# PASSIONLab/ELBA

Measured on AMD Instinct MI355X. Metric: overlap nnz/sec (A·Aᵀ SpGEMM, SharedSeeds semiring, after Prune(numshared<=1)), higher is better.
Workload: dtype u32

## Files before the change

### elba_amd/csrc/ov_plan.hpp

```cpp
#pragma once
#include <algorithm>
#include <cstddef>
#include <cstdint>

namespace elba {

constexpr int NUM_LDS_TIERS = 5;
constexpr int NUM_TIERS = NUM_LDS_TIERS + 1;
constexpr int LDS_TBITS0 = 9;
constexpr uint32_t STAGE_CHUNK = 1024;
constexpr uint32_t STAGE_REC_BYTES = 32;
constexpr uint32_t FIN_WAVE2_MAX = 1024;
constexpr uint32_t SLAB_PAD = 16;
constexpr int RP_TILE = 1024;
constexpr int FIN_HUGE_BLOCKS = 32;
constexpr int OV_SAMPLE_ROWS = 256, OV_SAMPLE_TIER = 3;
constexpr size_t OV_LDS_MAX = 160 * 1024;

namespace ov_spec {
constexpr uint32_t half = 1, inl = 1, pay16 = 1, rec16 = 1, suffix = 0, qblk_log2 = 0, j_shift = 0;
constexpr uint32_t hint_mask = 1u << 31, pos_mask = 0x3FFFFFFFu;
}

enum OvFamily { OV_DENSE, OV_PAY, OV_S32, OV_SHARED };
// ... 11 lines not shown
    {OV_PAY, 2, 512, 11, 0, 2, 26, false, true, false, 0},
    {OV_PAY, 3, 1024, 12, 0, 1, 26, false, true, false, 0},
    {OV_S32, 0, 128, 9, 0, 12, 18, false, false, false, 0},
    {OV_S32, 1, 256, 10, 0, 7, 18, false, false, false, 0},
    {OV_S32, 2, 512, 11, 0, 3, 18, false, false, false, 0},
    {OV_S32, 3, 1024, 12, 0, 1, 18, false, false, false, 0},
    {OV_SHARED, 4, 256, 13, 0, 1, 18, false, false, false, 0},
    {OV_SHARED, NUM_LDS_TIERS, 256, 0, 0, OV_GRID_SPILL, 0, true, false, false, 0},
};
constexpr int OV_NROWS = (int)(sizeof(OV_ROWS) / sizeof(OV_ROWS[0]));

constexpr int64_t ov_stage_slack(int num_cus) { return (int64_t)num_cus * 32 * STAGE_CHUNK + 64; }

constexpr size_t ov_row_lds(const OvTierRow &r, bool pay16)
{
    const size_t waves = (size_t)(r.block / 64), table = r.global ? 0 : (size_t)r.slot_bytes << r.tbits;
    return table + 256 + waves * (r.dense ? 2368 : r.global ? 2560 : r.payload ? 3072 : pay16 ? 2048 : 2560);
}

inline int ov_row_of(OvFamily family, int tier, int dense_up)
{
    int found = -1;
    for (int r = 0; r < OV_NROWS; ++r) {
        const OvTierRow &x = OV_ROWS[r];
        if (x.tier == tier && (x.family == family || x.family == OV_SHARED) && dense_up >= x.dense_up_min) found = r;
    }
    return found;
}

struct OvOptions {
    bool no_symmetry = false, no_pay = false, mir32 = false, no_slab = false, no_sample = false, ov_generic = false;
    int dk = -1, dense_up = 1, dense_wgs = 8, slab_q16 = 0, slab_pct = 175;
    int64_t tune3 = 0, tune4 = 0, tune5 = 0, tune7 = 0;
};
struct OvHints { uint32_t prior_q16 = 0, slab_q16 = 0; bool tiers_known = false, tier_used[NUM_TIERS] = {false, false, false, false, false, false}, sort_used[2] = {false, false}; };
struct OvInput {
    int64_t M = 0, N = 0, Z = 0, row_lo = 0, row_hi = 0, max_row_nnz = 0, max_col_nnz = 0;
    uint32_t fbits = 1;
    bool pos16 = false, use_ell = false, csr_hints = false, csr_inline = false, csr_suffix = false, have_row_order = false;
    int num_cus = 256;
    OvOptions opt;
    OvHints hints;
    int phase = 0, pass = 1;
    int64_t tmp_cap = 0, free_bytes = 0, workspace_hint_bytes = 0;
};

struct OvLaunch { int row = -1, grid = 0, block = 0; size_t lds = 0; };
struct OvFinPlan {
    int64_t nrows = 0;
    bool slabs = false, scan_rowptr = false, narrow = false;
    int slab_fold_blocks = 0, rowptr_blocks = 0, row_blocks = 0, bucket_blocks = 0, huge_blocks = FIN_HUGE_BLOCKS;
    uint64_t sort_stride = 2;
    uint32_t sorts = 0;
};
struct OvPlan {
    int64_t nrows = 0;
    bool whole = false, ell = false, forced = false;
    uint32_t half = 0, pos_mask = 0, hint_mask = 0, suffix = 0, inl = 0;
    bool row_order = false, hints_used = false;
    bool pay = false, pay16 = false;
    OvFamily family = OV_S32;
    int dk = 1;
    bool spec = false;
    uint32_t min_tier = 0, qblk_log2 = 0, prior_q16 = 16384, use_feedback = 1, max_col = 1;
    unsigned long long fb_enough = 0;
    uint32_t nsample = 0, sstep = 1;
    bool slab_on = false; int64_t slab_cap = 0; uint32_t slab_prior_q16 = 0;
    uint64_t gstride = 2; int spill_blocks = 64;
    int64_t slack = 0, tmp_cap = 0, b_cap = 0;
    bool mir16 = false;
    uint32_t tier_limit[NUM_LDS_TIERS] = {0, 0, 0, 0, 0};
    OvLaunch tier[NUM_TIERS], sample;
    int tmax = NUM_TIERS;
    uint32_t launched = 0;
    int zero_blocks_max = 0, classify_blocks = 0;
    OvFinPlan fin;
};

inline bool ov_spec_ok(const OvPlan &p)
{
    return !p.forced && p.dk == 0 && !p.pay && (p.pay16 ? 1u : 0u) == ov_spec::pay16 && p.ell && p.half == ov_spec::half && p.hint_mask == ov_spec::hint_mask &&
           p.pos_mask == ov_spec::pos_mask && p.inl == ov_spec::inl && (p.mir16 ? 1u : 0u) == ov_spec::rec16 && p.suffix == ov_spec::suffix && !p.row_order &&
           p.qblk_log2 == ov_spec::qblk_log2 && p.whole;
}

inline OvLaunch ov_launch_of(int row, bool pay16, int num_cus, int dense_wgs, int spill_blocks)
{
    const OvTierRow &r = OV_ROWS[row];
    OvLaunch l;
    l.row = row; l.block = r.block; l.lds = ov_row_lds(r, pay16);
    l.grid = r.cu_factor == OV_GRID_SPILL ? spill_blocks : num_cus * (r.cu_factor == OV_GRID_DENSE_WGS ? dense_wgs : r.cu_factor);
    return l;
}

inline OvFinPlan plan_ov_finalize(const OvInput &in, bool slabs, bool all_sorts, bool remote)
{
    OvFinPlan f;
    const int64_t M = in.M, cus = in.num_cus;
    f.nrows = in.row_hi - in.row_lo;
    f.slabs = slabs;
    f.slab_fold_blocks = slabs && f.nrows > 0 ? (int)((f.nrows + 255) / 256) : 0;
    while (f.sort_stride < (uint64_t)M) f.sort_stride <<= 1;
    f.scan_rowptr = M + 1 > (1 << 17);
    f.rowptr_blocks = (int)(f.scan_rowptr ? (M + 1 + 255) / 256 : (M + 1 + RP_TILE - 1) / RP_TILE);
    if (f.nrows <= 0) return f;
    f.row_blocks = (int)std::min<int64_t>((f.nrows + 3) / 4, cus * 32);
    f.narrow = in.opt.tune4 != 2 && !remote &&
               std::min<uint64_t>((uint64_t)std::max<int64_t>(in.max_row_nnz, 1) * (uint64_t)std::max<int64_t>(in.max_col_nnz, 1), (uint64_t)M) <= (uint64_t)FIN_WAVE2_MAX;
    f.bucket_blocks = (int)std::min<int64_t>(f.nrows, cus * 4);
    if (!f.narrow && (all_sorts || in.hints.sort_used[0])) f.sorts |= 1u;
    if (!f.narrow && (all_sorts || in.hints.sort_used[1])) f.sorts |= 2u;
    return f;
}

inline bool ov_one_triangle(const OvInput &in) { return in.phase >= 1 || !in.opt.no_symmetry || in.csr_inline; }

struct OvSpill { uint64_t gstride; int blocks; };
inline OvSpill ov_spill_tables(int64_t M, int num_cus)
{
    OvSpill s{2, 0};
    while (s.gstride < 2ull * (uint64_t)(M > 1 ? M : 1)) s.gstride <<= 1;
    s.blocks = (int)((4ull << 30) / (20ull * s.gstride));
    s.blocks = s.blocks < 64 ? 64 : (s.blocks > num_cus * 2 ? num_cus * 2 : s.blocks);
    return s;
}

inline void ov_plan_capacities(const OvInput &in, OvPlan &p)
{
    const int64_t M = in.M, Z = in.Z;
    const bool half = ov_one_triangle(in);
    const OvSpill sp = ov_spill_tables(M, in.num_cus);
    p.gstride = sp.gstride; p.spill_blocks = sp.blocks;
    p.slack = ov_stage_slack(in.num_cus);
    p.tmp_cap = in.tmp_cap;
    if (p.tmp_cap == 0) {
        if (in.workspace_hint_bytes > 0) p.tmp_cap = in.workspace_hint_bytes / (int64_t)STAGE_REC_BYTES;
        else {
            const int64_t budget = (int64_t)((size_t)in.free_bytes / 2 / (STAGE_REC_BYTES + (half ? 2 * (24 + 32) : 24)));
            p.tmp_cap = std::min<int64_t>(std::max<int64_t>(half ? Z / 2 : Z, 1 << 16) + p.slack, std::max<int64_t>(budget, 1024));
        }
        if (p.tmp_cap < 1024) p.tmp_cap = 1024;
    }
    p.b_cap = half ? 2 * p.tmp_cap : p.tmp_cap;
}

inline void ov_plan_switches(const OvInput &in, OvPlan &p)
{
    const OvOptions &o = in.opt;
    const int64_t Z = in.Z, nrows = p.nrows;
    p.max_col = (uint32_t)(in.max_col_nnz > 0 ? in.max_col_nnz : 1);
    p.half = in.phase >= 1 ? 2u : (ov_one_triangle(in) ? 1u : 0u);
    p.pos_mask = in.csr_suffix ? 0xFFFFu : (in.csr_hints ? 0x3FFFFFFFu : 0xFFFFFFFFu);
    p.hint_mask = !in.csr_hints ? 0u : (p.half == 2u ? 1u << 30 : (p.half == 1u ? 1u << 31 : 0u));
    p.suffix = in.csr_suffix && p.half == 1u ? 1u : 0u;
    p.inl = in.csr_inline ? 1u : 0u;
    p.row_order = p.suffix && in.have_row_order;
    p.hints_used = p.hint_mask != 0u || p.suffix != 0u || in.csr_inline;
    p.prior_q16 = in.hints.prior_q16 ? in.hints.prior_q16 : 16384u;
    p.use_feedback = in.hints.prior_q16 ? 0u : 1u;
    p.fb_enough = (unsigned long long)std::min<int64_t>(std::max<int64_t>(Z / 32, 1 << 16), 1 << 23);
    p.pay = in.pos16 && !o.no_pay;
    p.pay16 = p.pay && in.use_ell && !in.csr_suffix && o.tune3 != 1 && ((uint64_t)in.max_row_nnz << in.fbits) <= 65536ull;
// ... 96 lines not shown
```

### elba_amd/csrc/spgemm.hip

```cpp
#include "common.hpp"
#include "ov_plan.hpp"
#include <algorithm>
#include <string>
#include <type_traits>
#include <utility>

namespace elba {

namespace {

constexpr uint32_t EMPTY = 0xFFFFFFFFu;
constexpr uint32_t FIN_WAVE_MAX = 256;
constexpr uint32_t FIN_LDS_MAX = 4096;

struct alignas(128) OvShard {
    unsigned long long yraw, nnz, ndiag, nupper, fb_claims, fb_ub, products;
    unsigned int maxshared;
    unsigned int tier_done[NUM_TIERS];
};
constexpr int NUM_SHARDS = 64;

struct OvCounters {
    unsigned long long cursor;
    unsigned long long products;
// ... 74 lines not shown
    uint32_t tier_limit[NUM_LDS_TIERS];
    unsigned long long fb_enough, tmp_cap;
    uint32_t *row_cnt, *low_cnt; unsigned long long *row_off;
    uint32_t *lists, *sample_list;
    OvCounters *ctr;
    uint4 *rec; uint32_t *tick;
    uint4 *slab; unsigned long long *slab_pos;
};

struct ZeroList { uint32_t *p[6]; size_t words[6]; int n; };
__global__ __launch_bounds__(256) void k_zero_regions(ZeroList z)
{
    const size_t stride = (size_t)gridDim.x * 256u;
    for (int q = 0; q < z.n; ++q)
        for (size_t i = (size_t)blockIdx.x * 256u + threadIdx.x; i < z.words[q]; i += stride) z.p[q][i] = 0u;
}

struct __attribute__((packed, aligned(4))) RowPair { uint32_t a, b; };
__device__ __forceinline__ uint32_t slab_base(uint32_t rp, uint32_t rp0, uint32_t row_rel, uint32_t q16)
{
    return (uint32_t)(((unsigned long long)(rp - rp0) * q16) >> 16) + SLAB_PAD * row_rel;
}

__device__ __forceinline__ uint32_t wave_sum_u32(uint32_t v)
{
#pragma unroll
    for (int d = 32; d >= 1; d >>= 1) v += __shfl_xor(v, d, 64);
    return v;
}

__device__ __forceinline__ uint32_t guaranteed_tbits(uint32_t ub, uint32_t mcols)
{
    const uint32_t need = ub < mcols ? ub : mcols;
    return need <= 1 ? 1u : (uint32_t)(32 - __clz(2 * need - 1));
}

#include "spgemm_table.hpp"
#include "spgemm_direct.hpp"

struct FinParams {
    const uint32_t *row_cnt; uint32_t *low_cnt; const unsigned long long *row_off; int64_t *b_rowptr;
    const StageRec *tmp; StageRec *mir;
    uint32_t rec16; const uint4 *rec; const uint32_t *tick;
    uint32_t *b_col; elba_seed_t *b_val;
    uint32_t M, row_lo, row_hi, half;
    uint32_t *fin_lists; OvCounters *ctr;
    uint64_t *sortkeys; unsigned long long sort_stride;
    uint32_t *sum_tmp;
    long long b_cap;
    uint32_t mir16;
    const uint32_t *tick_rows;
    const uint32_t *a_rowptr; uint4 *slab;
    const unsigned long long *slab_pos; uint32_t *slab_n;
};

struct SlabCall { uint32_t q16, rp0; };
__device__ __forceinline__ SlabCall slab_call(const FinParams &p)
{
    SlabCall s{0u, 0u};
    if (p.slab) { s.q16 = p.ctr->slab_q16; if (s.q16) s.rp0 = p.a_rowptr[p.row_lo]; }
    return s;
}
__device__ __forceinline__ uint2 slab_row(const FinParams &p, const SlabCall &s, uint32_t i)
{
    if (!s.q16) return make_uint2(0u, 0u);
    return make_uint2(slab_base(p.a_rowptr[i], s.rp0, i - p.row_lo, s.q16), p.slab_n[i]);
}
__global__ void k_slab_fold(FinParams p)
{
    const uint32_t i = p.row_lo + blockIdx.x * blockDim.x + threadIdx.x;
    if (i >= p.row_hi) return;
    const SlabCall s = slab_call(p);
    uint32_t n = 0;
    if (s.q16) {
        const unsigned long long w = p.slab_pos[i];
        const uint32_t base = slab_base(p.a_rowptr[i], s.rp0, i - p.row_lo, s.q16), cur = (uint32_t)w, lim = (uint32_t)(w >> 32);
        n = (cur < lim ? cur : lim) - base;
    }
    p.slab_n[i] = n;
}

__device__ __forceinline__ void fin_load(const FinParams &p, uint32_t low, unsigned long long off, int64_t dst, uint32_t t, uint4 &a, uint4 &b, uint2 sl = make_uint2(0u, 0u))
{
    if (t >= low) {
        if (p.rec16) {
            const uint4 m = p.rec[off + (t - low)];
            a = make_uint4(m.x, 0xFFFFFFFFu, m.y & 0xFFFFu, m.y >> 16); b = make_uint4(m.z & 0xFFFFu, m.z >> 16, m.w, 0u);
        } else { const StageRec *r = &p.tmp[off + (t - low)]; a = r->a; b = r->b; }
    }
    else if (p.mir16) {
        const uint4 m = t < sl.y ? p.slab[sl.x + t] : reinterpret_cast<const uint4 *>(p.mir)[dst + t - sl.y];
        a = make_uint4(m.x, 0xFFFFFFFFu, m.y & 0xFFFFu, m.y >> 16); b = make_uint4(m.z & 0xFFFFu, m.z >> 16, m.w, 0u);
    } else { const StageRec *r = &p.mir[dst + t]; a = r->a; b = r->b; }
}
__device__ __forceinline__ uint32_t fin_col(const FinParams &p, uint32_t low, unsigned long long off, int64_t dst, uint32_t t, uint2 sl = make_uint2(0u, 0u))
{
    if (t >= low) return p.rec16 ? p.rec[off + (t - low)].x : p.tmp[off + (t - low)].a.x;
    return p.mir16 ? (t < sl.y ? p.slab[sl.x + t].x : reinterpret_cast<const uint4 *>(p.mir)[dst + t - sl.y].x) : p.mir[dst + t].a.x;
}
__device__ __forceinline__ elba_seed_t rec_seed(const uint4 a, const uint4 b)
{
    elba_seed_t v;
    v.q0 = a.z; v.t0 = a.w; v.q1 = b.x; v.t1 = b.y; v.numshared = (int32_t)b.z;
    return v;
}

__global__ __launch_bounds__(256) void k_row_pointers(FinParams p)
{
    __shared__ unsigned long long wsum[4], bsum;
    const uint32_t tid = threadIdx.x, lane = tid & 63, w = tid >> 6;
    const uint32_t n = p.M + 1, t0 = blockIdx.x * RP_TILE;
    unsigned long long pre = 0;
    {
        const uint4 *ca = reinterpret_cast<const uint4 *>(p.row_cnt), *cb = reinterpret_cast<const uint4 *>(p.low_cnt), *cc = reinterpret_cast<const uint4 *>(p.slab_n);
#pragma unroll 4
        for (uint32_t q = tid; q < t0 / 4; q += 256) {
            const uint4 x = ca[q], z = cb[q];
            pre += (unsigned long long)x.x + x.y + x.z + x.w + z.x + z.y + z.z + z.w;
            if (cc) { const uint4 y2 = cc[q]; pre += (unsigned long long)y2.x + y2.y + y2.z + y2.w; }
        }
    }
    uint32_t v[4];
    unsigned long long mine = 0;
#pragma unroll
    for (int u = 0; u < 4; ++u) {
        const uint32_t e = t0 + tid * 4 + u;
        v[u] = e < p.M ? p.row_cnt[e] + p.low_cnt[e] + (p.slab_n ? p.slab_n[e] : 0u) : 0u;
        mine += v[u];
    }
#pragma unroll
    for (int d = 32; d >= 1; d >>= 1) pre += __shfl_xor(pre, d, 64);
    unsigned long long inc = mine;
#pragma unroll
    for (int d = 1; d < 64; d <<= 1) { const unsigned long long o = __shfl_up(inc, d, 64); if ((int)lane >= d) inc += o; }
    if (lane == 63) wsum[w] = inc;
    if (tid == 0) bsum = 0;
    __syncthreads();
    if (lane == 0) atomicAdd(&bsum, pre);
    __syncthreads();
    unsigned long long run = bsum + inc - mine;
    for (uint32_t k = 0; k < w; ++k) run += wsum[k];
#pragma unroll
    for (int u = 0; u < 4; ++u) {
        const uint32_t e = t0 + tid * 4 + u;
        if (e < n) p.b_rowptr[e] = (int64_t)run;
        run += v[u];
    }
}

__global__ void k_sum_counts(FinParams p)
{
    const uint32_t e = blockIdx.x * blockDim.x + threadIdx.x;
    if (e <= p.M) p.sum_tmp[e] = e < p.M ? p.row_cnt[e] + p.low_cnt[e] + (p.slab_n ? p.slab_n[e] : 0u) : 0u;
}

__global__ __launch_bounds__(256) void k_mirror(FinParams p)
{
    const uint32_t lane = threadIdx.x & 63;
    const uint32_t wave = (blockIdx.x * blockDim.x + threadIdx.x) >> 6;
    const uint32_t nwaves = (gridDim.x * blockDim.x) >> 6;
    uint32_t placed = 0;
    for (uint32_t i = p.row_lo + wave; i < p.row_hi; i += nwaves) {
        const uint32_t own = p.row_cnt[i];
        const unsigned long long off = p.row_off[i];
        const uint32_t y = own + p.low_cnt[i] + (p.slab_n ? p.slab_n[i] : 0u);
        if (lane == 0 && y > FIN_WAVE2_MAX) {
            const int which = y > FIN_LDS_MAX ? 1 : 0;
            const uint32_t at = atomicAdd(&p.ctr->fin_count[which], 1u);
            p.fin_lists[(size_t)which * p.M + at] = i;
        }
        if (!p.half || p.rec16) continue;
        if (p.tick_rows && !((p.tick_rows[i >> 5] >> (i & 31u)) & 1u)) continue;
        for (uint32_t t = lane; t < own; t += 64) {
            const uint4 a = p.tmp[off + t].a;
            if (a.y == 0xFFFFFFFFu) continue;
            const uint4 b = p.tmp[off + t].b;
            const int64_t at = p.b_rowptr[a.x] + (int64_t)a.y;
            if (at >= p.b_cap) continue;
            if (p.mir16) reinterpret_cast<uint4 *>(p.mir)[at] = make_uint4(i, a.w | a.z << 16, b.y | b.x << 16, b.z);
            else {
                p.mir[at].a = make_uint4(i, 0xFFFFFFFFu, a.w, a.z);
                p.mir[at].b = make_uint4(b.y, b.x, b.z, 0u);
            }
        }
    }
    if (p.half && p.rec16) {
        const uint32_t n = p.ctr->ntick, stride = gridDim.x * blockDim.x;
        for (uint32_t e = blockIdx.x * blockDim.x + threadIdx.x; e < n; e += stride) {
            const uint32_t i = p.tick[3ull * e], t = p.tick[3ull * e + 1u], tk = p.tick[3ull * e + 2u];
            const uint4 r = p.rec[p.row_off[i] + t];
            const uint4 img = make_uint4(i, (r.y >> 16) | (r.y << 16), (r.z >> 16) | (r.z << 16), r.w);
            ++placed;
            const int64_t at = p.b_rowptr[r.x] + (int64_t)tk;
            if (at >= p.b_cap) continue;
            if (p.mir16) reinterpret_cast<uint4 *>(p.mir)[at] = img;
            else { p.mir[at].a = make_uint4(i, 0xFFFFFFFFu, img.y & 0xFFFFu, img.y >> 16); p.mir[at].b = make_uint4(img.z & 0xFFFFu, img.z >> 16, img.w, 0u); }
        }
    }
    placed = wave_sum_u32(placed);
    if (lane == 0 && placed) atomicAdd(&p.ctr->mir_placed, (unsigned long long)placed);
}

__global__ __launch_bounds__(256) void k_finalize_wave(FinParams p)
{
    __shared__ uint32_t colsm[4][FIN_WAVE_MAX];
    const int lane = threadIdx.x & 63, w = threadIdx.x >> 6;
    const uint32_t wave = (blockIdx.x * blockDim.x + threadIdx.x) >> 6;
    const uint32_t nwaves = (gridDim.x * blockDim.x) >> 6;
    uint32_t *cols = colsm[w];
    const SlabCall sc = slab_call(p);
    for (uint32_t i = p.row_lo + wave; i < p.row_hi; i += nwaves) {
        const int64_t dst = p.b_rowptr[i];
        const uint32_t y = (uint32_t)(p.b_rowptr[i + 1] - dst);
        const uint32_t lowt = p.low_cnt[i];
        if (lane == 0 && lowt) p.low_cnt[i] = 0;
        if (y == 0 || y > FIN_WAVE_MAX) continue;
        if (dst + (int64_t)y > p.b_cap) continue;
        const unsigned long long off = p.row_off[i];
        const uint2 sl = slab_row(p, sc, i);
        const uint32_t low = lowt + sl.y;
        uint32_t mine[4];
        uint4 ra[4], rb[4];
#pragma unroll
        for (int u = 0; u < 4; ++u) {
            const uint32_t t = (uint32_t)lane + 64u * u;
            mine[u] = 0xFFFFFFFFu;
            if (t < y) {
                fin_load(p, low, off, dst, t, ra[u], rb[u], sl);
                mine[u] = ra[u].x;
                cols[t] = mine[u];
            }
        }
        __builtin_amdgcn_fence(__ATOMIC_RELEASE, "wavefront");
        __builtin_amdgcn_wave_barrier();
        uint32_t rank[4] = {0, 0, 0, 0};
        for (uint32_t l = 0; l < y; ++l) {
            const uint32_t c = cols[l];
#pragma unroll
            for (int u = 0; u < 4; ++u) rank[u] += c < mine[u] ? 1u : 0u;
        }
#pragma unroll
        for (int u = 0; u < 4; ++u) {
            const uint32_t t = (uint32_t)lane + 64u * u;
            if (t < y) { p.b_col[dst + rank[u]] = mine[u]; p.b_val[dst + rank[u]] = rec_seed(ra[u], rb[u]); }
        }
        __builtin_amdgcn_wave_barrier();
    }
}

__global__ __launch_bounds__(256) void k_finalize_mid(FinParams p)
{
    __shared__ uint64_t lkeys[4][FIN_WAVE2_MAX];
    __shared__ uint32_t bst[4][128], bfl[4][128];
    const int lane = threadIdx.x & 63, w = threadIdx.x >> 6;
    const uint32_t wave = (blockIdx.x * blockDim.x + threadIdx.x) >> 6;
    const uint32_t nwaves = (gridDim.x * blockDim.x) >> 6;
    const SlabCall sc = slab_call(p);
    for (uint32_t i = p.row_lo + wave; i < p.row_hi; i += nwaves) {
        const int64_t dst = p.b_rowptr[i];
        const uint32_t y = (uint32_t)(p.b_rowptr[i + 1] - dst);
        if (y <= FIN_WAVE_MAX || y > FIN_WAVE2_MAX) continue;
        if (dst + (int64_t)y > p.b_cap) continue;
        const uint32_t low = y - p.row_cnt[i];
        const unsigned long long off = p.row_off[i];
        const uint2 sl = slab_row(p, sc, i);
        uint32_t nb = y / 8;
        nb = nb > 128u ? 128u : nb;
        const unsigned long long scale = ((unsigned long long)nb << 32) / (p.M > 0 ? p.M : 1u);
        bst[w][lane] = 0; bst[w][lane + 64] = 0; bfl[w][lane] = 0; bfl[w][lane + 64] = 0;
        __builtin_amdgcn_fence(__ATOMIC_RELEASE, "wavefront");
        __builtin_amdgcn_wave_barrier();
        uint32_t col[FIN_WAVE2_MAX / 64];
#pragma unroll
        for (int u = 0; u < (int)(FIN_WAVE2_MAX / 64); ++u) {
            const uint32_t t = (uint32_t)lane + 64u * u;
            col[u] = t < y ? fin_col(p, low, off, dst, t, sl) : 0u;
        }
#pragma unroll
        for (int u = 0; u < (int)(FIN_WAVE2_MAX / 64); ++u)
            if ((uint32_t)lane + 64u * u < y) atomicAdd(&bst[w][(uint32_t)(((unsigned long long)col[u] * scale) >> 32)], 1u);
        __builtin_amdgcn_fence(__ATOMIC_ACQ_REL, "wavefront");
        __builtin_amdgcn_wave_barrier();
        {
            const uint32_t c0 = bst[w][2 * lane], c1 = bst[w][2 * lane + 1];
            const uint32_t inc = wave_add_scan(c0 + c1);
            const uint32_t ex = inc - c0 - c1;
            __builtin_amdgcn_wave_barrier();
            bst[w][2 * lane] = ex; bst[w][2 * lane + 1] = ex + c0;
        }
        __builtin_amdgcn_fence(__ATOMIC_ACQ_REL, "wavefront");
        __builtin_amdgcn_wave_barrier();
#pragma unroll
        for (int u = 0; u < (int)(FIN_WAVE2_MAX / 64); ++u) {
            const uint32_t t = (uint32_t)lane + 64u * u;
            if (t < y) {
                const uint32_t b = (uint32_t)(((unsigned long long)col[u] * scale) >> 32);
                lkeys[w][bst[w][b] + atomicAdd(&bfl[w][b], 1u)] = ((uint64_t)col[u] << 32) | t;
            }
        }
        __builtin_amdgcn_fence(__ATOMIC_ACQ_REL, "wavefront");
        __builtin_amdgcn_wave_barrier();
        for (uint32_t e = (uint32_t)lane; e < y; e += 64u) {
            const uint64_t k = lkeys[w][e];
            const uint32_t c = (uint32_t)(k >> 32);
            const uint32_t b = (uint32_t)(((unsigned long long)c * scale) >> 32);
            const uint32_t lo = bst[w][b], hi = lo + bfl[w][b];
            uint4 ra, rb;
            fin_load(p, low, off, dst, (uint32_t)k, ra, rb, sl);
            uint32_t rank = 0;
            uint64_t kk[8];
#pragma unroll
            for (int q = 0; q < 8; ++q) kk[q] = lkeys[w][lo + (uint32_t)q < hi ? lo + (uint32_t)q : lo];
#pragma unroll
            for (int q = 0; q < 8; ++q) rank += (lo + (uint32_t)q < hi && kk[q] < k) ? 1u : 0u;
            for (uint32_t x = lo + 8u; x < hi; ++x) rank += lkeys[w][x] < k ? 1u : 0u;
            p.b_col[dst + lo + rank] = c;
            p.b_val[dst + lo + rank] = rec_seed(ra, rb);
        }
        __builtin_amdgcn_fence(__ATOMIC_ACQ_REL, "wavefront");
        __builtin_amdgcn_wave_barrier();
    }
}

__global__ __launch_bounds__(256, 3) void k_finalize_mid16(FinParams p)
{
    constexpr int NU = (int)(FIN_WAVE2_MAX / 64);
    __shared__ uint32_t lkeys[4][FIN_WAVE2_MAX];
    __shared__ uint32_t bst[4][128], bfl[4][128];
    __shared__ uint4 stage[4][256];
    const int lane = threadIdx.x & 63, w = threadIdx.x >> 6;
    const uint32_t wave = (blockIdx.x * blockDim.x + threadIdx.x) >> 6;
    const uint32_t nwaves = (gridDim.x * blockDim.x) >> 6;
    const uint4 *mir = reinterpret_cast<const uint4 *>(p.mir);
    const SlabCall sc = slab_call(p);
    for (uint32_t i = p.row_lo + wave; i < p.row_hi; i += nwaves) {
        const int64_t dst = p.b_rowptr[i];
        const uint32_t y = (uint32_t)(p.b_rowptr[i + 1] - dst);
        if (y <= FIN_WAVE_MAX || y > FIN_WAVE2_MAX) continue;
        if (dst + (int64_t)y > p.b_cap) continue;
        const uint32_t low = y - p.row_cnt[i];
        const unsigned long long off = p.row_off[i];
        uint2 sl = slab_row(p, sc, i);
        sl = make_uint2(sfirst(sl.x), sfirst(sl.y));
        uint32_t nb = y / 8;
        nb = nb > 128u ? 128u : nb;
        const unsigned long long scale = ((unsigned long long)nb << 32) / (p.M > 0 ? p.M : 1u);
        bst[w][lane] = 0; bst[w][lane + 64] = 0; bfl[w][lane] = 0; bfl[w][lane + 64] = 0;
        __builtin_amdgcn_fence(__ATOMIC_RELEASE, "wavefront");
        __builtin_amdgcn_wave_barrier();
        uint4 m[NU];
#pragma unroll
        for (int u = 0; u < NU; ++u) {
            const uint32_t t = (uint32_t)lane + 64u * u;
            m[u] = t < y ? (t >= low ? p.rec[off + (t - low)] : (t < sl.y ? p.slab[sl.x + t] : mir[dst + t - sl.y])) : make_uint4(0u, 0u, 0u, 0u);
        }
#pragma unroll
        for (int u = 0; u < NU; ++u)
            if ((uint32_t)lane + 64u * u < y) atomicAdd(&bst[w][(uint32_t)(((unsigned long long)m[u].x * scale) >> 32)], 1u);
        __builtin_amdgcn_fence(__ATOMIC_ACQ_REL, "wavefront");
        __builtin_amdgcn_wave_barrier();
        {
            const uint32_t c0 = bst[w][2 * lane], c1 = bst[w][2 * lane + 1];
            const uint32_t inc = wave_add_scan(c0 + c1);
            const uint32_t ex = inc - c0 - c1;
            __builtin_amdgcn_wave_barrier();
            bst[w][2 * lane] = ex; bst[w][2 * lane + 1] = ex + c0;
        }
        __builtin_amdgcn_fence(__ATOMIC_ACQ_REL, "wavefront");
        __builtin_amdgcn_wave_barrier();
#pragma unroll
        for (int u = 0; u < NU; ++u) {
            if ((uint32_t)lane + 64u * u < y) {
                const uint32_t b = (uint32_t)(((unsigned long long)m[u].x * scale) >> 32);
                lkeys[w][bst[w][b] + atomicAdd(&bfl[w][b], 1u)] = m[u].x;
            }
        }
        __builtin_amdgcn_fence(__ATOMIC_ACQ_REL, "wavefront");
        __builtin_amdgcn_wave_barrier();
#pragma unroll
        for (int u = 0; u < NU; ++u) {
            if ((uint32_t)lane + 64u * u < y) {
                const uint32_t c = m[u].x;
                const uint32_t b = (uint32_t)(((unsigned long long)c * scale) >> 32);
                const uint32_t lo = bst[w][b], hi = lo + bfl[w][b];
                uint32_t rank = 0, kk[8];
#pragma unroll
                for (int q = 0; q < 8; ++q) kk[q] = lkeys[w][lo + (uint32_t)q < hi ? lo + (uint32_t)q : lo];
#pragma unroll
                for (int q = 0; q < 8; ++q) rank += (lo + (uint32_t)q < hi && kk[q] < c) ? 1u : 0u;
                for (uint32_t x = lo + 8u; x < hi; ++x) rank += lkeys[w][x] < c ? 1u : 0u;
                m[u].w |= (lo + rank) << 22;
            }
        }
        for (uint32_t w0 = 0; w0 < y; w0 += 256u) {
#pragma unroll
            for (int u = 0; u < NU; ++u) {
                const uint32_t pos = (m[u].w >> 22) - w0;
                if ((uint32_t)lane + 64u * u < y && pos < 256u) stage[w][pos] = make_uint4(m[u].x, m[u].y, m[u].z, m[u].w & 0x3FFFFFu);
            }
            __builtin_amdgcn_fence(__ATOMIC_ACQ_REL, "wavefront");
            __builtin_amdgcn_wave_barrier();
#pragma unroll
            for (int q = 0; q < 4; ++q) {
                const uint32_t e = w0 + 64u * q + (uint32_t)lane;
                if (e < y) {
                    const uint4 r = stage[w][64u * q + (uint32_t)lane];
                    p.b_col[dst + e] = r.x;
                    p.b_val[dst + e] = rec_seed(make_uint4(r.x, 0xFFFFFFFFu, r.y & 0xFFFFu, r.y >> 16), make_uint4(r.z & 0xFFFFu, r.z >> 16, r.w, 0u));
                }
            }
            __builtin_amdgcn_fence(__ATOMIC_ACQ_REL, "wavefront");
            __builtin_amdgcn_wave_barrier();
        }
    }
}

template <int BLOCK>
__device__ __forceinline__ void bitonic_sort(uint64_t *keys, uint32_t n2)
{
    for (uint32_t k = 2; k <= n2; k <<= 1) {
        for (uint32_t j = k >> 1; j > 0; j >>= 1) {
            for (uint32_t t = threadIdx.x; t < n2; t += BLOCK) {
                const uint32_t ixj = t ^ j;
                if (ixj > t) {
                    const uint64_t a = keys[t], b = keys[ixj];
                    const bool up = (t & k) == 0;
                    if ((a > b) == up) { keys[t] = b; keys[ixj] = a; }
                }
            }
            __syncthreads();
        }
    }
}

constexpr uint32_t FIN_BUCKETS = 512;
__global__ __launch_bounds__(256) void k_finalize_bucket(FinParams p)
{
    __shared__ uint64_t lkeys[FIN_LDS_MAX];
    __shared__ uint32_t bstart[FIN_BUCKETS], bfill[FIN_BUCKETS];
    __shared__ unsigned long long scale_s;
    const uint32_t tid = threadIdx.x, lane = tid & 63;
    const uint32_t n = p.ctr->fin_count[0];
    for (uint32_t it = blockIdx.x; it < n; it += gridDim.x) {
        const uint32_t i = p.fin_lists[it];
        const int64_t dst = p.b_rowptr[i];
        const uint32_t y = (uint32_t)(p.b_rowptr[i + 1] - dst);
        if (dst + (int64_t)y > p.b_cap) continue;
        const uint32_t low = y - p.row_cnt[i];
        const unsigned long long off = p.row_off[i];
        const uint2 sl = slab_row(p, slab_call(p), i);
        uint32_t nb = y / 8;
        nb = nb < 1 ? 1u : (nb > FIN_BUCKETS ? FIN_BUCKETS : nb);
        if (tid == 0) scale_s = ((unsigned long long)nb << 32) / (p.M > 0 ? p.M : 1u);
        for (uint32_t b = tid; b < FIN_BUCKETS; b += 256) { bstart[b] = 0; bfill[b] = 0; }
        __syncthreads();
        const unsigned long long scale = scale_s;
        for (uint32_t t = tid; t < y; t += 256) {
            const uint32_t col = fin_col(p, low, off, dst, t, sl);
            atomicAdd(&bstart[(uint32_t)(((unsigned long long)col * scale) >> 32)], 1u);
        }
        __syncthreads();
        if (tid < 64) {
            uint32_t c[8], sum = 0;
#pragma unroll
            for (int u = 0; u < 8; ++u) { c[u] = bstart[lane * 8 + u]; sum += c[u]; }
            uint32_t inc = sum;
// ... 320 lines not shown
    if (r.plan.slab_on) add(c.ov_slabn.p, (size_t)(M + 8) * 4);
    size_t most = 0;
    for (int q = 0; q < z.n; ++q) most = std::max(most, z.words[q]);
    hipLaunchKernelGGL(k_zero_regions, dim3((unsigned)std::min<size_t>((most + 255) / 256, (size_t)r.plan.zero_blocks_max)), dim3(256), 0, c.stream, z);
    c.ov_low_clean = false;
}

static void ov_sample(OvRun &r)
{
    Ctx &c = r.c;
    const bool sampling = r.plan.sample.row >= 0;
    if (sampling) hipLaunchKernelGGL(k_classify_direct, dim3(1), dim3(256), 0, c.stream, r.p, 1);
    if (r.timed) c.ov_marks.mark(1, c.stream);
    if (!sampling) return;
    ov_launch(OvRowSeq{}, r.plan.sample, r.plan, r.p, c.stream, 1u);
    r.p.use_feedback = 0;
}

static void ov_classify(OvRun &r)
{
    if (r.plan.classify_blocks > 0) hipLaunchKernelGGL(k_classify_direct, dim3((unsigned)r.plan.classify_blocks), dim3(256), 0, r.c.stream, r.p, 0);
}

static void ov_numeric(OvRun &r)
{
    Ctx &c = r.c;
    c.ov_spec = r.plan.nrows > 0 && r.plan.spec ? 1 : 0;
    for (int t = 0; t < NUM_TIERS; ++t)
        if ((r.plan.launched >> t) & 1u) ov_launch(OvRowSeq{}, r.plan.tier[t], r.plan, r.p, c.stream, 0u);
    if (r.plan.nrows > 0) ELBA_HIP(hipGetLastError());
    if (r.timed) c.ov_marks.mark(2, c.stream);
}

static void ov_finalize(Ctx &c, const OvFinPlan &fp, uint32_t half, const StageRec *remote, int64_t nremote, int64_t slot = 0)
{
    hipStream_t s = c.stream;
    const int64_t M = c.M;
    const RowWindow w = c.window();
    const int cus = c.num_cus;
    const bool mir16 = ov_mir16(c);
    c.ov_sortkeys.reserve((size_t)fp.huge_blocks * fp.sort_stride * 8);
    if (fp.scan_rowptr) c.ov_sum_tmp.reserve((size_t)(M + 2) * 4);
    FinParams f{};
    f.row_cnt = c.ov_rowcnt.as<uint32_t>(); f.low_cnt = c.ov_totcnt.as<uint32_t>(); f.tmp = c.ov_tmp.as<StageRec>(); f.mir = half ? c.ov_mir.as<StageRec>() : nullptr; f.half = half; f.row_off = c.ov_rowoff.as<unsigned long long>(); f.b_rowptr = c.b_rowptr.as<int64_t>();
    f.b_col = c.b_col.as<uint32_t>(); f.b_val = c.b_val.as<elba_seed_t>();
    f.M = (uint32_t)M; f.row_lo = (uint32_t)w.lo; f.row_hi = (uint32_t)w.hi; f.fin_lists = c.ov_lists.as<uint32_t>() + (size_t)NUM_TIERS * (size_t)(M + 1); f.ctr = c.ov_counters.as<OvCounters>();
    f.b_cap = c.b_cap_entries;
    f.mir16 = mir16 ? 1u : 0u;
    f.tick_rows = c.ov_tickrows.as<uint32_t>();
    f.rec16 = c.ov_rec16 ? 1u : 0u; f.rec = c.ov_tmp.as<uint4>(); f.tick = reinterpret_cast<const uint32_t *>(c.ov_tmp.as<char>() + (size_t)c.ov_tmp_cap * 16);
    f.a_rowptr = c.a_rowptr.as<uint32_t>(); f.slab = fp.slabs ? c.ov_slab.as<uint4>() : nullptr;
    f.slab_pos = f.slab ? c.ov_slabpos.as<unsigned long long>() : nullptr; f.slab_n = f.slab ? c.ov_slabn.as<uint32_t>() : nullptr;
    f.sortkeys = c.ov_sortkeys.as<uint64_t>(); f.sort_stride = fp.sort_stride;
    if (fp.slab_fold_blocks > 0) hipLaunchKernelGGL(k_slab_fold, dim3((unsigned)fp.slab_fold_blocks), dim3(256), 0, s, f);
    if (!fp.scan_rowptr) hipLaunchKernelGGL(k_row_pointers, dim3((unsigned)fp.rowptr_blocks), dim3(256), 0, s, f);
    else {
        f.sum_tmp = c.ov_sum_tmp.as<uint32_t>();
        hipLaunchKernelGGL(k_sum_counts, dim3((unsigned)fp.rowptr_blocks), dim3(256), 0, s, f);
        exclusive_scan_u32_to_i64(s, f.sum_tmp, c.b_rowptr.as<int64_t>(), M + 1, c.ws_scan);
    }
    if (fp.nrows <= 0) return;
    const dim3 rows((unsigned)fp.row_blocks);
    hipLaunchKernelGGL(k_mirror, rows, dim3(256), 0, s, f);
    if (nremote > 0 && slot == 0) hipLaunchKernelGGL(k_place_remote, dim3((unsigned)std::min<int64_t>((nremote + 255) / 256, (int64_t)cus * 32)), dim3(256), 0, s, f, remote, (unsigned long long)nremote, 0ull);
    if (nremote > 0 && slot != 0) hipLaunchKernelGGL(k_place_remote, dim3((unsigned)std::min<int64_t>((slot + 255) / 256, (int64_t)cus * 4), (unsigned)(nremote / slot)), dim3(256), 0, s, f, remote, (unsigned long long)nremote, (unsigned long long)slot);
    hipLaunchKernelGGL(k_finalize_wave, rows, dim3(256), 0, s, f);
    if (f.rec16 && f.mir16) hipLaunchKernelGGL(k_finalize_mid16, rows, dim3(256), 0, s, f);
    else hipLaunchKernelGGL(k_finalize_mid, rows, dim3(256), 0, s, f);
    if (fp.sorts & 1u) hipLaunchKernelGGL(k_finalize_bucket, dim3((unsigned)fp.bucket_blocks), dim3(256), 0, s, f);
    if (fp.sorts & 2u) hipLaunchKernelGGL(k_finalize_huge, dim3((unsigned)fp.huge_blocks), dim3(256), 0, s, f);
}

static void ov_read_back(OvRun &r)
{
    Ctx &c = r.c;
    if (r.timed) c.ov_marks.mark(3, c.stream);
    ELBA_HIP(hipMemcpyAsync(r.hc, c.ov_counters.p, sizeof(OvCounters), hipMemcpyDeviceToHost, c.stream));
    ELBA_HIP(hipStreamSynchronize(c.stream));
    if (r.timed) { r.ms_sym += c.ov_marks.ms(0, 1); r.ms_num += c.ov_marks.ms(1, 2); r.ms_fin = c.ov_marks.ms(2, 3); r.ms_tot += c.ov_marks.ms(0, 3); }
    r.was_timed = r.timed;
    c.ov_passes = r.passes; c.ov_forwarded += r.hc->nforward;
}

static bool ov_settle(OvRun &r)
{
    Ctx &c = r.c;
    const OvCounters &hc = *r.hc;
    const uint32_t sorts = r.in.phase == 0 ? r.plan.fin.sorts : 3u;
    bool missed = false;
    for (int t = 0; t < NUM_TIERS; ++t) missed |= !((r.plan.launched >> t) & 1u) && hc.tier_count[t] > 0;
    missed |= (!(sorts & 1u) && hc.fin_count[0] > 0) || (!(sorts & 2u) && hc.fin_count[1] > 0);
    if (!hc.overflow && !missed) { c.ov_low_clean = r.in.phase == 0; return true; }
    if (c.opt.trace) fprintf(stderr, "[elba] overlap call repeated: overflow=%u missed=%d cursor=%llu tmp_cap=%lld\n", hc.overflow, (int)missed, hc.cursor, (long long)c.ov_tmp_cap);
    ELBA_REQUIRE(r.passes < 4, ELBA_ERR_INTERNAL, "overlap output did not settle");
    c.ov_tiers_known = false;
    r.in = ov_next_pass(r.in, r.plan, hc.overflow != 0, hc.cursor);
    r.plan = plan_ov(r.in);
    ov_bind(r);
    return false;
}

static void ov_finish(Ctx &c, OvCounters &hc, int passes, bool was_timed, float ms_tot, float ms_sym, float ms_num, float ms_fin, int64_t extra_nnz, int64_t extra_upper)
{
    const int64_t M = c.M, N = c.N, Z = c.Z;
    const RowWindow w = c.window();
    elba_overlap_stats st{};
    st.nrows = w.rows();
#ifdef ELBA_PHASE_CLOCK
    fprintf(stderr, "[elba phase] wave-0 cycles summed over %llu workgroups: header=%llu init=%llu accumulate=%llu handoff=%llu sweep=%llu reserve=%llu store=%llu | rows %u,%u,%u,%u,%u,%u\n",
            hc.phase[10], hc.phase[0], hc.phase[1], hc.phase[2], hc.phase[3], hc.phase[4], hc.phase[5], hc.phase[6],
            hc.tier_count[0], hc.tier_count[1], hc.tier_count[2], hc.tier_count[3], hc.tier_count[4], hc.tier_count[5]);
#endif
    OvMeasured m;
    for (int sh = 0; sh < NUM_SHARDS; ++sh) {
        const OvShard &x = hc.shard[sh];
        hc.yraw += x.yraw; hc.nnz += x.nnz; hc.ndiag += x.ndiag; hc.nupper += x.nupper; hc.products += x.products;
        if (x.maxshared > hc.maxshared) hc.maxshared = x.maxshared;
        for (int t = 0; t < NUM_TIERS; ++t) hc.tier_done[t] += x.tier_done[t];
        m.fb_claims += x.fb_claims; m.fb_ub += x.fb_ub;
// ... 300 lines not shown
```

Before: 17.16 billion.

## Restructure finalize pipeline: fold slab counts into sum, split mirror, merge small-row finalize

Folds the slab-fill computation into the row-count summation kernel when a scan is used, and moves the large-row queueing out of the mirror kernel into the row-pointer and sum kernels. The mirror kernel is split into a row-based variant and a tick-based variant, each launched only when needed. When the average row length is large it skips the wave-finalize kernel and lets the mid16 kernel handle small rows, using templated narrower register footprints and a padded-sentinel rank loop. The aim is fewer launches and less redundant work, at the cost of more complex control flow and some kernel-ordering subtleties, such as where low_cnt gets reset.

```diff
diff --git a/elba_amd/csrc/ov_plan.hpp b/elba_amd/csrc/ov_plan.hpp
--- a/elba_amd/csrc/ov_plan.hpp
+++ b/elba_amd/csrc/ov_plan.hpp
@@ -87,6 +87,9 @@
     int slab_fold_blocks = 0, rowptr_blocks = 0, row_blocks = 0, bucket_blocks = 0, huge_blocks = FIN_HUGE_BLOCKS;
     uint64_t sort_stride = 2;
     uint32_t sorts = 0;
+    bool fold_in_sum = false;
+    bool one_sort = false;
+    int tick_blocks = 0;
 };
 struct OvPlan {
     int64_t nrows = 0;
@@ -143,6 +146,9 @@
     f.narrow = in.opt.tune4 != 2 && !remote &&
                std::min<uint64_t>((uint64_t)std::max<int64_t>(in.max_row_nnz, 1) * (uint64_t)std::max<int64_t>(in.max_col_nnz, 1), (uint64_t)M) <= (uint64_t)FIN_WAVE2_MAX;
     f.bucket_blocks = (int)std::min<int64_t>(f.nrows, cus * 4);
+    f.fold_in_sum = slabs && f.scan_rowptr;
+    f.one_sort = in.Z / f.nrows >= 1024;
+    f.tick_blocks = (int)std::min<int64_t>(f.row_blocks, cus * 16);
     if (!f.narrow && (all_sorts || in.hints.sort_used[0])) f.sorts |= 1u;
     if (!f.narrow && (all_sorts || in.hints.sort_used[1])) f.sorts |= 2u;
     return f;
diff --git a/elba_amd/csrc/spgemm.hip b/elba_amd/csrc/spgemm.hip
--- a/elba_amd/csrc/spgemm.hip
+++ b/elba_amd/csrc/spgemm.hip
@@ -150,6 +150,7 @@
     const uint32_t *tick_rows;
     const uint32_t *a_rowptr; uint4 *slab;
     const unsigned long long *slab_pos; uint32_t *slab_n;
+    uint32_t fin_small;
 };
 
 struct SlabCall { uint32_t q16, rp0; };
@@ -164,18 +165,26 @@
     if (!s.q16) return make_uint2(0u, 0u);
     return make_uint2(slab_base(p.a_rowptr[i], s.rp0, i - p.row_lo, s.q16), p.slab_n[i]);
 }
+__device__ __forceinline__ uint32_t slab_fill(const FinParams &p, const SlabCall &s, uint32_t i)
+{
+    if (!s.q16) return 0u;
+    const unsigned long long w = p.slab_pos[i];
+    const uint32_t base = slab_base(p.a_rowptr[i], s.rp0, i - p.row_lo, s.q16), cur = (uint32_t)w, lim = (uint32_t)(w >> 32);
+    return (cur < lim ? cur : lim) - base;
+}
 __global__ void k_slab_fold(FinParams p)
 {
     const uint32_t i = p.row_lo + blockIdx.x * blockDim.x + threadIdx.x;
     if (i >= p.row_hi) return;
-    const SlabCall s = slab_call(p);
-    uint32_t n = 0;
-    if (s.q16) {
-        const unsigned long long w = p.slab_pos[i];
-        const uint32_t base = slab_base(p.a_rowptr[i], s.rp0, i - p.row_lo, s.q16), cur = (uint32_t)w, lim = (uint32_t)(w >> 32);
-        n = (cur < lim ? cur : lim) - base;
-    }
-    p.slab_n[i] = n;
+    p.slab_n[i] = slab_fill(p, slab_call(p), i);
+}
+
+__device__ __forceinline__ void fin_queue(const FinParams &p, uint32_t i, uint32_t y)
+{
+    if (y <= FIN_WAVE2_MAX || i < p.row_lo || i >= p.row_hi) return;
+    const int which = y > FIN_LDS_MAX ? 1 : 0;
+    const uint32_t at = atomicAdd(&p.ctr->fin_count[which], 1u);
+    p.fin_lists[(size_t)which * p.M + at] = i;
 }
 
 __device__ __forceinline__ void fin_load(const FinParams &p, uint32_t low, unsigned long long off, int64_t dst, uint32_t t, uint4 &a, uint4 &b, uint2 sl = make_uint2(0u, 0u))
@@ -225,6 +234,7 @@
         const uint32_t e = t0 + tid * 4 + u;
         v[u] = e < p.M ? p.row_cnt[e] + p.low_cnt[e] + (p.slab_n ? p.slab_n[e] : 0u) : 0u;
         mine += v[u];
+        fin_queue(p, e, v[u]);
     }
 #pragma unroll
     for (int d = 32; d >= 1; d >>= 1) pre += __shfl_xor(pre, d, 64);
@@ -249,26 +259,29 @@
 __global__ void k_sum_counts(FinParams p)
 {
     const uint32_t e = blockIdx.x * blockDim.x + threadIdx.x;
-    if (e <= p.M) p.sum_tmp[e] = e < p.M ? p.row_cnt[e] + p.low_cnt[e] + (p.slab_n ? p.slab_n[e] : 0u) : 0u;
-}
-
-__global__ __launch_bounds__(256) void k_mirror(FinParams p)
+    if (e > p.M) return;
+    uint32_t y = 0;
+    if (e < p.M) {
+        uint32_t sn = 0;
+        if (p.slab_n) {
+            if (e >= p.row_lo && e < p.row_hi) { sn = slab_fill(p, slab_call(p), e); p.slab_n[e] = sn; }
+            else sn = p.slab_n[e];
+        }
+        y = p.row_cnt[e] + p.low_cnt[e] + sn;
+        fin_queue(p, e, y);
+    }
+    p.sum_tmp[e] = y;
+}
+
+__global__ __launch_bounds__(256) void k_mirror_rows(FinParams p)
 {
     const uint32_t lane = threadIdx.x & 63;
     const uint32_t wave = (blockIdx.x * blockDim.x + threadIdx.x) >> 6;
     const uint32_t nwaves = (gridDim.x * blockDim.x) >> 6;
-    uint32_t placed = 0;
     for (uint32_t i = p.row_lo + wave; i < p.row_hi; i += nwaves) {
+        if (p.tick_rows && !((p.tick_rows[i >> 5] >> (i & 31u)) & 1u)) continue;
         const uint32_t own = p.row_cnt[i];
         const unsigned long long off = p.row_off[i];
-        const uint32_t y = own + p.low_cnt[i] + (p.slab_n ? p.slab_n[i] : 0u);
-        if (lane == 0 && y > FIN_WAVE2_MAX) {
-            const int which = y > FIN_LDS_MAX ? 1 : 0;
-            const uint32_t at = atomicAdd(&p.ctr->fin_count[which], 1u);
-            p.fin_lists[(size_t)which * p.M + at] = i;
-        }
-        if (!p.half || p.rec16) continue;
-        if (p.tick_rows && !((p.tick_rows[i >> 5] >> (i & 31u)) & 1u)) continue;
         for (uint32_t t = lane; t < own; t += 64) {
             const uint4 a = p.tmp[off + t].a;
             if (a.y == 0xFFFFFFFFu) continue;
@@ -282,18 +295,21 @@
             }
         }
     }
-    if (p.half && p.rec16) {
-        const uint32_t n = p.ctr->ntick, stride = gridDim.x * blockDim.x;
-        for (uint32_t e = blockIdx.x * blockDim.x + threadIdx.x; e < n; e += stride) {
-            const uint32_t i = p.tick[3ull * e], t = p.tick[3ull * e + 1u], tk = p.tick[3ull * e + 2u];
-            const uint4 r = p.rec[p.row_off[i] + t];
-            const uint4 img = make_uint4(i, (r.y >> 16) | (r.y << 16), (r.z >> 16) | (r.z << 16), r.w);
-            ++placed;
-            const int64_t at = p.b_rowptr[r.x] + (int64_t)tk;
-            if (at >= p.b_cap) continue;
-            if (p.mir16) reinterpret_cast<uint4 *>(p.mir)[at] = img;
-            else { p.mir[at].a = make_uint4(i, 0xFFFFFFFFu, img.y & 0xFFFFu, img.y >> 16); p.mir[at].b = make_uint4(img.z & 0xFFFFu, img.z >> 16, img.w, 0u); }
-        }
+}
+__global__ __launch_bounds__(256) void k_mirror_ticks(FinParams p)
+{
+    const uint32_t lane = threadIdx.x & 63;
+    uint32_t placed = 0;
+    const uint32_t n = p.ctr->ntick, stride = gridDim.x * blockDim.x;
+    for (uint32_t e = blockIdx.x * blockDim.x + threadIdx.x; e < n; e += stride) {
+        const uint32_t i = p.tick[3ull * e], t = p.tick[3ull * e + 1u], tk = p.tick[3ull * e + 2u];
+        const uint4 r = p.rec[p.row_off[i] + t];
+        const uint4 img = make_uint4(i, (r.y >> 16) | (r.y << 16), (r.z >> 16) | (r.z << 16), r.w);
+        ++placed;
+        const int64_t at = p.b_rowptr[r.x] + (int64_t)tk;
+        if (at >= p.b_cap) continue;
+        if (p.mir16) reinterpret_cast<uint4 *>(p.mir)[at] = img;
+        else { p.mir[at].a = make_uint4(i, 0xFFFFFFFFu, img.y & 0xFFFFu, img.y >> 16); p.mir[at].b = make_uint4(img.z & 0xFFFFu, img.z >> 16, img.w, 0u); }
     }
     placed = wave_sum_u32(placed);
     if (lane == 0 && placed) atomicAdd(&p.ctr->mir_placed, (unsigned long long)placed);
@@ -310,13 +326,11 @@
     for (uint32_t i = p.row_lo + wave; i < p.row_hi; i += nwaves) {
         const int64_t dst = p.b_rowptr[i];
         const uint32_t y = (uint32_t)(p.b_rowptr[i + 1] - dst);
-        const uint32_t lowt = p.low_cnt[i];
-        if (lane == 0 && lowt) p.low_cnt[i] = 0;
         if (y == 0 || y > FIN_WAVE_MAX) continue;
         if (dst + (int64_t)y > p.b_cap) continue;
         const unsigned long long off = p.row_off[i];
         const uint2 sl = slab_row(p, sc, i);
-        const uint32_t low = lowt + sl.y;
+        const uint32_t low = y - p.row_cnt[i];
         uint32_t mine[4];
         uint4 ra[4], rb[4];
 #pragma unroll
@@ -344,6 +358,11 @@
         }
         __builtin_amdgcn_wave_barrier();
     }
+}
+
+__device__ __forceinline__ void fin_hand_back(const FinParams &p, uint32_t i, int lane)
+{
+    if (lane == 0 && p.low_cnt[i]) p.low_cnt[i] = 0;
 }
 
 __global__ __launch_bounds__(256) void k_finalize_mid(FinParams p)
@@ -357,6 +376,7 @@
     for (uint32_t i = p.row_lo + wave; i < p.row_hi; i += nwaves) {
         const int64_t dst = p.b_rowptr[i];
         const uint32_t y = (uint32_t)(p.b_rowptr[i + 1] - dst);
+        fin_hand_back(p, i, lane);
         if (y <= FIN_WAVE_MAX || y > FIN_WAVE2_MAX) continue;
         if (dst + (int64_t)y > p.b_cap) continue;
         const uint32_t low = y - p.row_cnt[i];
@@ -420,96 +440,134 @@
     }
 }
 
+#ifndef ELBA_FIN_NARROW
+#define ELBA_FIN_NARROW 1
+#endif
+#ifndef ELBA_FIN_RANK_OPEN
+#define ELBA_FIN_RANK_OPEN 1
+#endif
+constexpr uint32_t FIN_RANK_AHEAD = 8;
+template <int NU>
+__device__ __forceinline__ void fin_row16(const FinParams &p, const uint4 *mir, int64_t dst, uint32_t y, uint32_t low, unsigned long long off, uint2 sl,
+                                          uint32_t *lkeys, uint32_t *bst, uint32_t *bfl, uint4 *stage, int lane)
+{
+    static_assert(FIN_RANK_AHEAD == 8, "the rank step reads eight keys ahead");
+    uint32_t nb = y / 8;
+    nb = nb > 128u ? 128u : nb;
+    const unsigned long long scale = ((unsigned long long)nb << 32) / (p.M > 0 ? p.M : 1u);
+    bst[lane] = 0; bst[lane + 64] = 0; bfl[lane] = 0; bfl[lane + 64] = 0;
+    __builtin_amdgcn_fence(__ATOMIC_RELEASE, "wavefront");
+    __builtin_amdgcn_wave_barrier();
+    uint4 m[NU];
+#pragma unroll
+    for (int u = 0; u < NU; ++u) {
+        const uint32_t t = (uint32_t)lane + 64u * u;
+        m[u] = t < y ? (t >= low ? p.rec[off + (t - low)] : (t < sl.y ? p.slab[sl.x + t] : mir[dst + t - sl.y])) : make_uint4(0u, 0u, 0u, 0u);
+    }
+#pragma unroll
+    for (int u = 0; u < NU; ++u)
+        if ((uint32_t)lane + 64u * u < y) atomicAdd(&bst[(uint32_t)(((unsigned long long)m[u].x * scale) >> 32)], 1u);
+    __builtin_amdgcn_fence(__ATOMIC_ACQ_REL, "wavefront");
+    __builtin_amdgcn_wave_barrier();
+    {
+        const uint32_t c0 = bst[2 * lane], c1 = bst[2 * lane + 1];
+        const uint32_t inc = wave_add_scan(c0 + c1);
+        const uint32_t ex = inc - c0 - c1;
+        __builtin_amdgcn_wave_barrier();
+        bst[2 * lane] = ex; bst[2 * lane + 1] = ex + c0;
+    }
+    __builtin_amdgcn_fence(__ATOMIC_ACQ_REL, "wavefront");
+    __builtin_amdgcn_wave_barrier();
+#pragma unroll
+    for (int u = 0; u < NU; ++u) {
+        if ((uint32_t)lane + 64u * u < y) {
+            const uint32_t b = (uint32_t)(((unsigned long long)m[u].x * scale) >> 32);
+            lkeys[bst[b] + atomicAdd(&bfl[b], 1u)] = m[u].x;
+        }
+    }
+#if ELBA_FIN_RANK_OPEN
+    if ((uint32_t)lane < FIN_RANK_AHEAD) lkeys[y + (uint32_t)lane] = 0xFFFFFFFFu;
+#endif
+    __builtin_amdgcn_fence(__ATOMIC_ACQ_REL, "wavefront");
+    __builtin_amdgcn_wave_barrier();
+#pragma unroll
+    for (int u = 0; u < NU; ++u) {
+        if ((uint32_t)lane + 64u * u < y) {
+            const uint32_t c = m[u].x;
+            const uint32_t b = (uint32_t)(((unsigned long long)c * scale) >> 32);
+            const uint32_t lo = bst[b];
+            uint32_t rank = 0, kk[8];
+#if !ELBA_FIN_RANK_OPEN
+            const uint32_t hi = lo + bfl[b];
+#endif
+#if ELBA_FIN_RANK_OPEN
+#pragma unroll
+            for (int q = 0; q < 8; ++q) kk[q] = lkeys[lo + (uint32_t)q];
+#pragma unroll
+            for (int q = 0; q < 8; ++q) rank += kk[q] < c ? 1u : 0u;
+#else
+#pragma unroll
+            for (int q = 0; q < 8; ++q) kk[q] = lkeys[lo + (uint32_t)q < hi ? lo + (uint32_t)q : lo];
+#pragma unroll
+            for (int q = 0; q < 8; ++q) rank += (lo + (uint32_t)q < hi && kk[q] < c) ? 1u : 0u;
+#endif
+#if ELBA_FIN_RANK_OPEN
+            for (uint32_t x = 8u, n = bfl[b]; x < n; ++x) rank += lkeys[lo + x] < c ? 1u : 0u;
+#else
+            for (uint32_t x = lo + 8u; x < hi; ++x) rank += lkeys[x] < c ? 1u : 0u;
+#endif
+            m[u].w |= (lo + rank) << 22;
+        }
+    }
+    for (uint32_t w0 = 0; w0 < y; w0 += 256u) {
+#pragma unroll
+        for (int u = 0; u < NU; ++u) {
+            const uint32_t pos = (m[u].w >> 22) - w0;
+            if ((uint32_t)lane + 64u * u < y && pos < 256u) stage[pos] = make_uint4(m[u].x, m[u].y, m[u].z, m[u].w & 0x3FFFFFu);
+        }
+        __builtin_amdgcn_fence(__ATOMIC_ACQ_REL, "wavefront");
+        __builtin_amdgcn_wave_barrier();
+#pragma unroll
+        for (int q = 0; q < 4; ++q) {
+            const uint32_t e = w0 + 64u * q + (uint32_t)lane;
+            if (e < y) {
+                const uint4 r = stage[64u * q + (uint32_t)lane];
+                p.b_col[dst + e] = r.x;
+                p.b_val[dst + e] = rec_seed(make_uint4(r.x, 0xFFFFFFFFu, r.y & 0xFFFFu, r.y >> 16), make_uint4(r.z & 0xFFFFu, r.z >> 16, r.w, 0u));
+            }
+        }
+        __builtin_amdgcn_fence(__ATOMIC_ACQ_REL, "wavefront");
+        __builtin_amdgcn_wave_barrier();
+    }
+}
+
 __global__ __launch_bounds__(256, 3) void k_finalize_mid16(FinParams p)
 {
-    constexpr int NU = (int)(FIN_WAVE2_MAX / 64);
-    __shared__ uint32_t lkeys[4][FIN_WAVE2_MAX];
+    __shared__ uint32_t lkeys[4][FIN_WAVE2_MAX + FIN_RANK_AHEAD];
     __shared__ uint32_t bst[4][128], bfl[4][128];
     __shared__ uint4 stage[4][256];
-    const int lane = threadIdx.x & 63, w = threadIdx.x >> 6;
+    const int lane = threadIdx.x & 63, w = (int)sfirst(threadIdx.x >> 6);
     const uint32_t wave = (blockIdx.x * blockDim.x + threadIdx.x) >> 6;
     const uint32_t nwaves = (gridDim.x * blockDim.x) >> 6;
     const uint4 *mir = reinterpret_cast<const uint4 *>(p.mir);
     const SlabCall sc = slab_call(p);
+    const uint32_t ymin = p.fin_small ? 0u : FIN_WAVE_MAX;
     for (uint32_t i = p.row_lo + wave; i < p.row_hi; i += nwaves) {
-        const int64_t dst = p.b_rowptr[i];
-        const uint32_t y = (uint32_t)(p.b_rowptr[i + 1] - dst);
-        if (y <= FIN_WAVE_MAX || y > FIN_WAVE2_MAX) continue;
+        const int64_t dst = (int64_t)sfirst64((uint64_t)p.b_rowptr[i]);
+        const uint32_t y = sfirst((uint32_t)(p.b_rowptr[i + 1] - dst));
+        fin_hand_back(p, i, lane);
+        if (y <= ymin || y > FIN_WAVE2_MAX) continue;
         if (dst + (int64_t)y > p.b_cap) continue;
-        const uint32_t low = y - p.row_cnt[i];
-        const unsigned long long off = p.row_off[i];
+        const uint32_t low = y - sfirst(p.row_cnt[i]);
+        const unsigned long long off = sfirst64(p.row_off[i]);
         uint2 sl = slab_row(p, sc, i);
         sl = make_uint2(sfirst(sl.x), sfirst(sl.y));
-        uint32_t nb = y / 8;
-        nb = nb > 128u ? 128u : nb;
-        const unsigned long long scale = ((unsigned long long)nb << 32) / (p.M > 0 ? p.M : 1u);
-        bst[w][lane] = 0; bst[w][lane + 64] = 0; bfl[w][lane] = 0; bfl[w][lane + 64] = 0;
-        __builtin_amdgcn_fence(__ATOMIC_RELEASE, "wavefront");
-        __builtin_amdgcn_wave_barrier();
-        uint4 m[NU];
-#pragma unroll
-        for (int u = 0; u < NU; ++u) {
-            const uint32_t t = (uint32_t)lane + 64u * u;
-            m[u] = t < y ? (t >= low ? p.rec[off + (t - low)] : (t < sl.y ? p.slab[sl.x + t] : mir[dst + t - sl.y])) : make_uint4(0u, 0u, 0u, 0u);
-        }
-#pragma unroll
-        for (int u = 0; u < NU; ++u)
-            if ((uint32_t)lane + 64u * u < y) atomicAdd(&bst[w][(uint32_t)(((unsigned long long)m[u].x * scale) >> 32)], 1u);
-        __builtin_amdgcn_fence(__ATOMIC_ACQ_REL, "wavefront");
-        __builtin_amdgcn_wave_barrier();
-        {
-            const uint32_t c0 = bst[w][2 * lane], c1 = bst[w][2 * lane + 1];
-            const uint32_t inc = wave_add_scan(c0 + c1);
-            const uint32_t ex = inc - c0 - c1;
-            __builtin_amdgcn_wave_barrier();
-            bst[w][2 * lane] = ex; bst[w][2 * lane + 1] = ex + c0;
-        }
-        __builtin_amdgcn_fence(__ATOMIC_ACQ_REL, "wavefront");
-        __builtin_amdgcn_wave_barrier();
-#pragma unroll
-        for (int u = 0; u < NU; ++u) {
-            if ((uint32_t)lane + 64u * u < y) {
-                const uint32_t b = (uint32_t)(((unsigned long long)m[u].x * scale) >> 32);
-                lkeys[w][bst[w][b] + atomicAdd(&bfl[w][b], 1u)] = m[u].x;
-            }
-        }
-        __builtin_amdgcn_fence(__ATOMIC_ACQ_REL, "wavefront");
-        __builtin_amdgcn_wave_barrier();
-#pragma unroll
-        for (int u = 0; u < NU; ++u) {
-            if ((uint32_t)lane + 64u * u < y) {
-                const uint32_t c = m[u].x;
-                const uint32_t b = (uint32_t)(((unsigned long long)c * scale) >> 32);
-                const uint32_t lo = bst[w][b], hi = lo + bfl[w][b];
-                uint32_t rank = 0, kk[8];
-#pragma unroll
-                for (int q = 0; q < 8; ++q) kk[q] = lkeys[w][lo + (uint32_t)q < hi ? lo + (uint32_t)q : lo];
-#pragma unroll
-                for (int q = 0; q < 8; ++q) rank += (lo + (uint32_t)q < hi && kk[q] < c) ? 1u : 0u;
-                for (uint32_t x = lo + 8u; x < hi; ++x) rank += lkeys[w][x] < c ? 1u : 0u;
-                m[u].w |= (lo + rank) << 22;
-            }
-        }
-        for (uint32_t w0 = 0; w0 < y; w0 += 256u) {
-#pragma unroll
-            for (int u = 0; u < NU; ++u) {
-                const uint32_t pos = (m[u].w >> 22) - w0;
-                if ((uint32_t)lane + 64u * u < y && pos < 256u) stage[w][pos] = make_uint4(m[u].x, m[u].y, m[u].z, m[u].w & 0x3FFFFFu);
-            }
-            __builtin_amdgcn_fence(__ATOMIC_ACQ_REL, "wavefront");
-            __builtin_amdgcn_wave_barrier();
-#pragma unroll
-            for (int q = 0; q < 4; ++q) {
-                const uint32_t e = w0 + 64u * q + (uint32_t)lane;
-                if (e < y) {
-                    const uint4 r = stage[w][64u * q + (uint32_t)lane];
-                    p.b_col[dst + e] = r.x;
-                    p.b_val[dst + e] = rec_seed(make_uint4(r.x, 0xFFFFFFFFu, r.y & 0xFFFFu, r.y >> 16), make_uint4(r.z & 0xFFFFu, r.z >> 16, r.w, 0u));
-                }
-            }
-            __builtin_amdgcn_fence(__ATOMIC_ACQ_REL, "wavefront");
-            __builtin_amdgcn_wave_barrier();
-        }
+#if ELBA_FIN_NARROW
+        if (y <= 256u) fin_row16<4>(p, mir, dst, y, low, off, sl, lkeys[w], bst[w], bfl[w], stage[w], lane);
+        else if (y <= 512u) fin_row16<8>(p, mir, dst, y, low, off, sl, lkeys[w], bst[w], bfl[w], stage[w], lane);
+        else
+#endif
+        fin_row16<(int)(FIN_WAVE2_MAX / 64)>(p, mir, dst, y, low, off, sl, lkeys[w], bst[w], bfl[w], stage[w], lane);
     }
 }
 
@@ -936,7 +994,8 @@
     f.a_rowptr = c.a_rowptr.as<uint32_t>(); f.slab = fp.slabs ? c.ov_slab.as<uint4>() : nullptr;
     f.slab_pos = f.slab ? c.ov_slabpos.as<unsigned long long>() : nullptr; f.slab_n = f.slab ? c.ov_slabn.as<uint32_t>() : nullptr;
     f.sortkeys = c.ov_sortkeys.as<uint64_t>(); f.sort_stride = fp.sort_stride;
-    if (fp.slab_fold_blocks > 0) hipLaunchKernelGGL(k_slab_fold, dim3((unsigned)fp.slab_fold_blocks), dim3(256), 0, s, f);
+    f.fin_small = fp.one_sort && f.rec16 && f.mir16 ? 1u : 0u;
+    if (fp.slab_fold_blocks > 0 && !fp.fold_in_sum) hipLaunchKernelGGL(k_slab_fold, dim3((unsigned)fp.slab_fold_blocks), dim3(256), 0, s, f);
     if (!fp.scan_rowptr) hipLaunchKernelGGL(k_row_pointers, dim3((unsigned)fp.rowptr_blocks), dim3(256), 0, s, f);
     else {
         f.sum_tmp = c.ov_sum_tmp.as<uint32_t>();
@@ -945,10 +1004,11 @@
     }
     if (fp.nrows <= 0) return;
     const dim3 rows((unsigned)fp.row_blocks);
-    hipLaunchKernelGGL(k_mirror, rows, dim3(256), 0, s, f);
+    if (half && f.rec16) hipLaunchKernelGGL(k_mirror_ticks, dim3((unsigned)fp.tick_blocks), dim3(256), 0, s, f);
+    else if (half) hipLaunchKernelGGL(k_mirror_rows, rows, dim3(256), 0, s, f);
     if (nremote > 0 && slot == 0) hipLaunchKernelGGL(k_place_remote, dim3((unsigned)std::min<int64_t>((nremote + 255) / 256, (int64_t)cus * 32)), dim3(256), 0, s, f, remote, (unsigned long long)nremote, 0ull);
     if (nremote > 0 && slot != 0) hipLaunchKernelGGL(k_place_remote, dim3((unsigned)std::min<int64_t>((slot + 255) / 256, (int64_t)cus * 4), (unsigned)(nremote / slot)), dim3(256), 0, s, f, remote, (unsigned long long)nremote, (unsigned long long)slot);
-    hipLaunchKernelGGL(k_finalize_wave, rows, dim3(256), 0, s, f);
+    if (!f.fin_small) hipLaunchKernelGGL(k_finalize_wave, rows, dim3(256), 0, s, f);
     if (f.rec16 && f.mir16) hipLaunchKernelGGL(k_finalize_mid16, rows, dim3(256), 0, s, f);
     else hipLaunchKernelGGL(k_finalize_mid, rows, dim3(256), 0, s, f);
     if (fp.sorts & 1u) hipLaunchKernelGGL(k_finalize_bucket, dim3((unsigned)fp.bucket_blocks), dim3(256), 0, s, f);
```

Result: slower. 16.83 billion (-1.9%).
